# JTtNinjaCode/CPU-Ray-Tracing-Implementation

Hardware: AMD Instinct MI355X
Metric: Msamples/sec (pixels*spp) Cornell Box 800x800@1024spp; 1/2/4/8-GPU scaling (higher is better)
Workload: dtype fp64; 1 GPU; cornell_box 800x800 1024spp depth 50, light sampling on; key=cornell_box 800x800 1024spp depth 50 f64 pool=0 chunk=0 K=0 world=1, spp=1024, max_depth=50, tiles=16x16 round-robin over ranks, parallelism=tiles1, kernel_timing=on, rounds_per_frame=1, grid_lanes=458752

## Files before the change

### cpu-ray-tracing-implementation_amd/csrc/rt_device.h

```cpp
#pragma once

#include <hip/hip_runtime.h>
#include <stdint.h>

#include <type_traits>

#include "rt_scene.h"
#include "rt_sin.h"
#include "rt_types.h"

namespace rtd {

#ifndef RT_BIG_SPHERE_R
#define RT_BIG_SPHERE_R 16
#endif
#define RT_EXT_FN __device__ __attribute__((noinline))

#ifndef RT_PRECISE_F32
__device__ __forceinline__ float fdiv(float a, float b) { return a * __builtin_amdgcn_rcpf(b); }
__device__ __forceinline__ float fsqrt(float x) { return __builtin_amdgcn_sqrtf(x); }
__device__ __forceinline__ float flog(float x) { return __builtin_amdgcn_logf(x) * 0.693147180559945309f; }
__device__ __forceinline__ float frsq(float x) { return __builtin_amdgcn_rsqf(x); }
__device__ __forceinline__ void sincos2pi(float u, float& s, float& c) {
  s = __builtin_amdgcn_sinf(u);
  c = __builtin_amdgcn_cosf(u);
}
#else
__device__ __forceinline__ float fdiv(float a, float b) { return a / b; }
__device__ __forceinline__ float fsqrt(float x) { return sqrtf(x); }
__device__ __forceinline__ float flog(float x) { return logf(x); }
__device__ __forceinline__ float frsq(float x) { return 1.0f / sqrtf(x); }
__device__ __forceinline__ void sincos2pi(float u, float& s, float& c) {
  float phi = 2 * 3.14159265358979f * u;
  s = sinf(phi);
  c = cosf(phi);
}
#endif
__device__ __forceinline__ double frcp(double b) {
  const double r0 = __builtin_amdgcn_rcp(b);
// ... 1316 lines not shown
__device__ __forceinline__ void flat_quads(const FlatQuadT<R>* q, uint32_t n, int32_t base, V<R> o, V<R> d,
                                           V<R> inv, R tmin, R& tmax, int32_t& best, uint64_t xkey) {
#pragma unroll 1
  for (uint32_t k = 0; k + 1 < n; k += 2) {
    const FlatQuad2<R> r = ld_scalar(reinterpret_cast<const FlatQuad2<R>*>(q + k));
    flat_quad_test<A>(r.a, base + (int32_t)k, o, d, inv, tmin, tmax, best, xkey);
    flat_quad_test<A>(r.b, base + (int32_t)k + 1, o, d, inv, tmin, tmax, best, xkey);
  }
  if (n & 1u) flat_quad_test<A>(ld_scalar(q + (n - 1)), base + (int32_t)(n - 1), o, d, inv, tmin, tmax, best, xkey);
}
template <class R>
struct Slab {
  R t0[3], t1[3], tn, tf, th;
};
template <class R>
__device__ __forceinline__ Slab<R> flat_slab(const FlatBoxT<R>& b, V<R> o, V<R> inv, R tmin, int32_t excl_i,
                                             uint32_t xf) {
  Slab<R> s;
  const bool left = sizeof(R) == 4 && excl_i == b.inst;
  const R ninf = -Num<R>::inf();
  auto dist = [&](R p, R oa, R ia) { return (p - oa) * ia; };
  s.t0[0] = (left & (xf == 0)) ? ninf : dist(b.lo[0], o.x, inv.x);
  s.t1[0] = (left & (xf == 1)) ? ninf : dist(b.hi[0], o.x, inv.x);
  s.t0[1] = (left & (xf == 2)) ? ninf : dist(b.lo[1], o.y, inv.y);
  s.t1[1] = (left & (xf == 3)) ? ninf : dist(b.hi[1], o.y, inv.y);
  s.t0[2] = (left & (xf == 4)) ? ninf : dist(b.lo[2], o.z, inv.z);
  s.t1[2] = (left & (xf == 5)) ? ninf : dist(b.hi[2], o.z, inv.z);
  s.tn = fmax(fmax(fmin(s.t0[0], s.t1[0]), fmin(s.t0[1], s.t1[1])), fmin(s.t0[2], s.t1[2]));
  s.tf = fmin(fmin(fmax(s.t0[0], s.t1[0]), fmax(s.t0[1], s.t1[1])), fmax(s.t0[2], s.t1[2]));
  s.th = s.tn >= tmin ? s.tn : s.tf;
  return s;
}
template <class R>
__device__ __forceinline__ void trace_flat(const DevScene<R>& sc, V<R> o, V<R> d, uint32_t excl_e, int32_t excl_i,
                                           R& t_best, uint32_t& e_best, int32_t& i_best, uint32_t& nm,
                                           const FlatQuadT<R>* fq, const FlatBoxT<R>* fb) {
  const R tmin = R(0.001);
  R tmax = Num<R>::inf();
  const V<R> inv = flat_inv(d);
  const uint64_t xkey = ((uint64_t)(uint32_t)excl_i << 32) | excl_e;
  const uint32_t xf = excl_e & 7u;
  int32_t best = -1;
  const uint32_t n0 = sc.n_flatq[0], n1 = sc.n_flatq[1], n2 = sc.n_flatq[2], nq = n0 + n1 + n2;
  flat_quads<0>(sc.flatq, n0, 0, o, d, inv, tmin, tmax, best, xkey);
  flat_quads<1>(sc.flatq + n0, n1, (int32_t)n0, o, d, inv, tmin, tmax, best, xkey);
  flat_quads<2>(sc.flatq + n0 + n1, n2, (int32_t)(n0 + n1), o, d, inv, tmin, tmax, best, xkey);
#pragma unroll 1
  for (uint32_t k = 0; k < sc.n_flatb; k++) {
    const FlatBoxT<R> b = ld_scalar(sc.flatb + k);
    const Slab<R> s = flat_slab(b, o, inv, tmin, excl_i, xf);
    const bool h = (s.tf >= fmax(s.tn, tmin)) & (s.th <= tmax);
    tmax = h ? s.th : tmax;
    best = h ? (int32_t)(nq + k) : best;
  }
  t_best = tmax;
  e_best = kNoHit;
  i_best = -1;
  nm = 0;
  if (best < 0) return;
  if ((uint32_t)best < nq) {
    const FlatQuadT<R>& r = fq[best];
    e_best = r.e;
    i_best = r.inst;
    nm = r.nm;
    return;
  }
  const FlatBoxT<R>& b = fb[(uint32_t)best - nq];
  const Slab<R> s = flat_slab(b, o, inv, tmin, excl_i, xf);
  const bool enter = s.tn >= tmin;
  int k = 2;
  if (enter) {
    if (s.tn == fmin(s.t0[0], s.t1[0])) k = 0;
    else if (s.tn == fmin(s.t0[1], s.t1[1])) k = 1;
  } else {
    if (s.tf == fmax(s.t0[0], s.t1[0])) k = 0;
    else if (s.tf == fmax(s.t0[1], s.t1[1])) k = 1;
  }
  const R dk = k == 0 ? d.x : (k == 1 ? d.y : d.z);
  const int side = enter ? (dk < R(0) ? 1 : 0) : (dk < R(0) ? 0 : 1);
  e_best = b.face[2 * k + side];
  i_best = b.inst;
  nm = b.mat | (uint32_t)k << 28 | ((b.neg >> (2 * k + side)) & 1u) << 31;
}

__device__ __forceinline__ double perlin_noise(const double* tb, double px, double py, double pz) {
#pragma clang fp contract(off)
  int iu = (int)floor(px), iv = (int)floor(py), iw = (int)floor(pz);
  const double u = px - iu, v = py - iv, w = pz - iw;
  iu &= 255;
  iv &= 255;
  iw &= 255;
  const double* perm = tb + 3 * kPerlinPoints;
  const double uu = u * u * (3 - 2 * u), vv = v * v * (3 - 2 * v), ww = w * w * (3 - 2 * w);
  double accum = 0.0;
  for (int i = 0; i < 2; i++)
    for (int j = 0; j < 2; j++)
      for (int k = 0; k < 2; k++) {
        const int g = (int)perm[(iu + i) % 256] ^ (int)perm[(iv + j) % 256] ^ (int)perm[(iw + k) % 256];
        const double* r = tb + 3 * g;
        const double d = r[0] * (u - i) + r[1] * (v - j) + r[2] * (w - k);
// ... 266 lines not shown
```

### cpu-ray-tracing-implementation_amd/csrc/rt_kernels.hip

```cpp
#include <hip/hip_runtime.h>

#include <algorithm>
#include <cmath>
#include <map>
#include <mutex>
#include <tuple>

#include "../../include/rt_hip.h"
#include "rt_device.h"
#include "rt_launch.h"

using namespace rtd;

namespace {

#ifndef RT_LINEAR_WAVES
#define RT_LINEAR_WAVES 6
#endif
#ifndef RT_STACK_WAVES
#define RT_STACK_WAVES 4
#endif
#ifndef RT_LINEAR_WAVES_F64
#define RT_LINEAR_WAVES_F64 3
#endif
// ... 719 lines not shown
  static constexpr int kWaves = sizeof(R) != 4 ? (VOL ? RT_LINEAR_VOL_WAVES_F64 : RT_LINEAR_WAVES_F64)
                                 : (!SPH && !TRI && !VOL) ? RT_LINEAR_WAVES
                                 : (!SPH && !TRI && VOL)  ? (LLI ? RT_LINEAR_VOL_WAVES_LLI : RT_LINEAR_VOL_WAVES)
                                                          : 1;
  static constexpr bool kNoRad = VOL;
  static constexpr bool kColdLds = VOL;
  static constexpr bool kThrLds = VOL && LLI && sizeof(R) == 4;
  template <class PS>
  __device__ __forceinline__ static void run(const DevScene<R>& sc, const Node<R>*, const PS& s, Keys k,
                                             uint32_t*, R& t, uint32_t& e, int32_t& i, uint32_t&) {
    trace_linear<R, SPH, TRI, VOL>(sc, s.o, s.d, s.tm, s.xe, s.xi, k, (uint32_t)s.bounce, t, e, i);
  }
};
#ifndef RT_FLAT_WAVES
#define RT_FLAT_WAVES 8
#endif
#ifndef RT_FLAT_WAVES_F64
#define RT_FLAT_WAVES_F64 5
#endif
#ifndef RT_FLAT_WAVES_F64_LL
#define RT_FLAT_WAVES_F64_LL 7
#endif
template <class R, bool TLDS = false, bool LL = false>
struct FlatTrav : TravDefaults {
  static constexpr bool kFlat = true;
  static constexpr bool kTablesLds = TLDS;
  static constexpr bool kLL = LL;
  static constexpr int kWaves = sizeof(R) == 4 ? RT_FLAT_WAVES : (LL ? RT_FLAT_WAVES_F64_LL : RT_FLAT_WAVES_F64);
  static constexpr bool kNoRad = true;
  static constexpr bool kColdLds = sizeof(R) == 8;
  template <class PS>
  __device__ __forceinline__ static void run(const DevScene<R>& sc, const Node<R>*, const PS& s, Keys, uint32_t*,
                                             R& t, uint32_t& e, int32_t& i, uint32_t& nm) {
    trace_flat<R>(sc, s.o, s.d, s.xe, s.xi, t, e, i, nm, sc.flatq, sc.flatb);
  }
  static constexpr uint32_t kLdsQuads = LL ? 16 : 64, kLdsBoxes = LL ? 8 : 16, kLdsMats = LL ? 16 : 32;
  struct Tables {
    FlatQuadT<R> q[kLdsQuads];
    FlatBoxT<R> b[kLdsBoxes];
    Material<R> m[LL ? 1 : kLdsMats];
    R4<R> lm[LL ? kLdsMats : 1];
  };
  __host__ __device__ __forceinline__ static bool tables_fit(const DevScene<R>& sc) {
    return sc.n_flatq[0] + sc.n_flatq[1] + sc.n_flatq[2] <= kLdsQuads && sc.n_flatb <= kLdsBoxes &&
           sc.n_mats <= kLdsMats;
  }
  __device__ __forceinline__ static void fill(const DevScene<R>& sc, Tables& tb) {
    const uint32_t nq = sc.n_flatq[0] + sc.n_flatq[1] + sc.n_flatq[2];
    for (uint32_t j = threadIdx.x; j < nq; j += kBlock) tb.q[j] = sc.flatq[j];
    for (uint32_t j = threadIdx.x; j < sc.n_flatb; j += kBlock) tb.b[j] = sc.flatb[j];
    for (uint32_t j = threadIdx.x; j < sc.n_mats; j += kBlock) {
      if constexpr (LL) {
        const Material<R>& m = sc.mats[j];
        tb.lm[j] = R4<R>{m.tx.c0[0], m.tx.c0[1], m.tx.c0[2], m.kind == M_DIFFUSE_LIGHT ? R(1) : R(0)};
      } else {
        tb.m[j] = sc.mats[j];
      }
    }
  }
  template <class PS>
  __device__ __forceinline__ static void run_lds(const DevScene<R>& sc, const Tables& tb, const PS& s, R& t,
                                                 uint32_t& e, int32_t& i, uint32_t& nm) {
    trace_flat<R>(sc, s.o, s.d, s.xe, s.xi, t, e, i, nm, tb.q, tb.b);
  }
};
constexpr uint32_t kLdsNodeMax = 256;
template <class R, int STACK, bool LDSN = false>
struct StackTrav : TravDefaults {
  static constexpr int kStack = STACK;
  static constexpr int kLdsNodes = LDSN ? (int)kLdsNodeMax : 0;
  static constexpr int kWaves = sizeof(R) == 4 ? RT_STACK_WAVES : (LDSN ? 1 : RT_STACK_WAVES_F64);
  template <class PS>
  __device__ __forceinline__ static void run(const DevScene<R>& sc, const Node<R>* nodes, const PS& s, Keys k,
                                             uint32_t* stk, R& t, uint32_t& e, int32_t& i, uint32_t&) {
    trace<R, STACK, kBlock>(sc, LDSN ? nodes : sc.nodes, s.o, s.d, s.tm, s.xe, s.xi, k, (uint32_t)s.bounce, s.xy(),
                            stk, t, e, i);
  }
};

#ifndef RT_WIDE_WAVES
#define RT_WIDE_WAVES 7
#endif
#ifndef RT_SHADE_BATCH
#define RT_SHADE_BATCH 48
#endif
#ifndef RT_SHADE_BATCH_GLOBAL
#define RT_SHADE_BATCH_GLOBAL 48
#endif
#ifndef RT_WIDE_WAVES_F64
#define RT_WIDE_WAVES_F64 4
#endif
#ifndef RT_WIDE_WAVES_GLOBAL_F64
#define RT_WIDE_WAVES_GLOBAL_F64 4
#endif
#ifndef RT_WIDE_WAVES_GLOBAL_F64_LL
#define RT_WIDE_WAVES_GLOBAL_F64_LL 5
// ... 1074 lines not shown
```

### cpu-ray-tracing-implementation_amd/csrc/rt_render.hip

```cpp
#include <hip/hip_runtime.h>

#include <algorithm>
#include <chrono>
#include <cstdio>
#include <cstdlib>
#include <cstring>
#include <mutex>
#include <new>
#include <stdexcept>
#include <string>
#include <vector>

#include "../../include/rt_hip.h"
#include "rt_launch.h"
#include "rt_plan.h"
#include "scene_compile.h"

using namespace rtd;

struct DevBuf {
  void* ptr = nullptr;
  size_t bytes = 0;
};

// ... 120 lines not shown
    float a = 0;
    RT_HIP(c, hipEventElapsedTime(&a, c->events[k], c->events[k + 1]));
    ms += a;
  }
  c->ev_used = 0;
  c->last.step_ms += ms;
  uint32_t fault = 0;
  if (c->fault.ptr) RT_HIP(c, hipMemcpy(&fault, c->fault.ptr, 4, hipMemcpyDeviceToHost));
  if (fault) return set_err(c, RT_ERR_HIP, "a path did not finish (internal error)");
  return RT_OK;
}

template <class R>
DevScene<R> dev_scene(const SceneHeader& h, void* base) {
  auto at = [&](uint64_t off) { return (const unsigned char*)base + off; };
  DevScene<R> s{};
  s.quads = (const Quad<R>*)at(h.off_quads);
  s.spheres = (const Sphere<R>*)at(h.off_spheres);
  s.tris = (const Tri<R>*)at(h.off_tris);
  s.insts = (const Instance<R>*)at(h.off_instances);
  s.vols = (const Volume<R>*)at(h.off_volumes);
  s.nodes = (const Node<R>*)at(h.off_nodes);
  s.refs = (const uint32_t*)at(h.off_refs);
  s.mats = (const Material<R>*)at(h.off_mats);
  s.texs = (const Texture<R>*)at(h.off_texs);
  s.light = (const Light<R>*)at(h.off_light);
  s.lin = (const LinRec<R>*)at(h.off_linear);
  s.n_linear = h.n_linear;
  s.has_flat = (int32_t)h.has_flat;
  s.flatq = (const FlatQuadT<R>*)at(h.off_flat_quad);
  s.flatb = (const FlatBoxT<R>*)at(h.off_flat_box);
  for (int a = 0; a < 3; a++) s.n_flatq[a] = h.n_flat_quad[a];
  s.n_flatb = h.n_flat_box;
  s.n_mats = h.n_mats;
  s.root = h.root;
  s.background = h.background;
  s.has_volumes = h.has_volumes;
  s.n_nodes = h.n_nodes;
  s.texdata = (const double*)at(h.off_texdata);
  s.images = (const uint8_t*)at(h.off_images);
  s.has_procedural = h.n_texdata > 0 || h.has_cell_noise;
  s.has_wide = (int32_t)h.has_wide;
  s.wnodes = (const WNode*)at(h.off_wnodes);
  s.wprims = (const typename WWord<R>::T*)at(h.off_wprims);
  s.n_wnodes = h.n_wnodes;
  s.n_wprim_words = h.n_wprim_words;
  s.wroot = h.wroot;
  s.wide_stack = h.wide_stack;
  s.wide_kinds = h.wide_kinds;
  s.wide_big = h.wide_big;
  s.wide_top = h.wide_top;
  s.wnodesh = h.has_wnodesh ? (const WNodeH*)at(h.off_wnodesh) : nullptr;
  s.quads64 = h.has_quads64 ? (const Quad<double>*)at(h.off_quads64) : nullptr;
  return s;
}

template <class R>
rt_status wide_spill_area(rt_context* c, const SceneHeader& hdr, DevScene<R>& sc) {
  const uint32_t wide_need = hdr.wide_stack;
  constexpr uint32_t kWideLdsStack = wide_lds_stack<R>();
  if (hdr.has_wide && wide_need > kWideLdsStack) {
    int ncu = 0;
    RT_HIP(c, hipDeviceGetAttribute(&ncu, hipDeviceAttributeMultiprocessorCount, c->device));
    const uint32_t lanes = (uint32_t)std::max(ncu, 1) * 2048u;
    rt_status s;
    if ((s = ensure(c, c->wide_spill, 4ull * (wide_need - kWideLdsStack) * lanes)) != RT_OK) return s;
// ... 728 lines not shown
```

### cpu-ray-tracing-implementation_amd/csrc/rt_scene.h

```cpp
#pragma once

#include <stdint.h>

#if !defined(__HIP__) && !defined(__host__)
#define __host__
#define __device__
#endif

namespace rtd {

enum : uint32_t {
  E_QUAD = 0u,
  E_SPHERE = 1u,
  E_TRI = 2u,
  E_INSTANCE = 3u,
  E_VOLUME = 4u,
  E_NODE = 5u,
  E_LIST = 6u,
  E_SPECIAL = 7u,
};
constexpr uint32_t kTypeShift = 29;
constexpr uint32_t kPayloadMask = (1u << kTypeShift) - 1u;
constexpr uint32_t kEnd = (E_SPECIAL << kTypeShift) | 0u;
constexpr uint32_t kRestoreBase = (E_SPECIAL << kTypeShift) | 1u;
// ... 8 lines not shown
constexpr int kMaxBvhDepth = 26;
constexpr int kLinearMax = 96;
constexpr uint32_t kInstEnd = kRestoreBase;

template <class R>
struct alignas(16) LinRec {
  uint32_t op;
  uint32_t aux;
  R f[14];
};
static_assert(3 * kMaxChain <= 14, "an instance chain must fit one LinRec");

template <class R>
struct alignas(16) FlatQuadT {
  R plane, lo_u, lo_w, inv_u;
  R inv_w;
  uint32_t e;
  int32_t inst;
  uint32_t nm;
};
using FlatQuad = FlatQuadT<float>;
constexpr uint32_t kNmMat = (1u << 28) - 1u;
template <class R>
struct alignas(16) FlatBoxT {
  R lo[3];
  R hi[3];
  int32_t inst;
  uint32_t mat;
  uint32_t face[6];
  uint32_t neg;
  uint32_t pad;
};
using FlatBox = FlatBoxT<float>;
static_assert(sizeof(FlatQuadT<float>) == 32 && sizeof(FlatQuadT<double>) == 64, "flat quad records");
static_assert(sizeof(FlatBoxT<float>) == 64 && sizeof(FlatBoxT<double>) == 96, "flat box records");

template <class R>
struct alignas(16) Quad {
  R n[3];
  R D;
  R q[3];
  int32_t mat;
  R a[3];
  R area;
  R b[3];
  R pad;
};

template <class R>
struct alignas(16) Sphere {
  R c1[3];
  R r;
  R dc[3];
  int32_t mat;
  R cn[3];
  int32_t moving;
};

template <class R>
struct alignas(16) Tri {
  R p0[3];
  int32_t mat;
  R e1[3];
  R pad1;
  R e2[3];
  R pad2;
  R n[3];
// ... 105 lines not shown
  int32_t has_volumes;
  int32_t num_instances;
  uint64_t off_quads, off_spheres, off_tris, off_instances, off_volumes, off_nodes, off_refs, off_mats, off_texs,
      off_light, off_linear;
  uint64_t off_texdata;
  uint64_t n_texdata;
  int32_t has_cell_noise;
  int32_t pad2_;
  uint64_t off_images;
  uint64_t n_images;
  uint64_t bytes;
  uint32_t n_linear;
  uint32_t n_flat_box;
  uint32_t n_flat_quad[3];
  uint32_t has_flat;
  uint64_t off_flat_quad, off_flat_box;
  uint32_t n_quads, n_spheres, n_tris, n_volumes, n_nodes, n_refs, n_mats, n_texs;
  uint64_t off_wnodes, off_wprims;
  uint32_t n_wnodes, n_wprim_words;
  uint32_t wroot;
  uint32_t wide_stack;
  uint32_t wide_kinds;
  uint32_t has_wide;
  uint32_t wide_big;
  uint32_t has_wnodesh;
  uint64_t off_wnodesh;
  uint32_t has_quads64;
  uint64_t off_quads64;
  uint32_t mat_kinds;
  uint32_t tex_kinds;
  int32_t light_kind;
  int32_t light_aligned;
  uint32_t wide_top;
};

}
```

### cpu-ray-tracing-implementation_amd/csrc/rt_types.h

```cpp
#pragma once

#include <hip/hip_runtime.h>
#include <stdint.h>

#include "rt_scene.h"

namespace rtd {

template <class R>
struct V {
  R x, y, z;
};

__host__ __device__ __forceinline__ uint32_t mix32(uint32_t x) {
  x ^= x >> 16;
  x *= 0x21f0aaadu;
  x ^= x >> 15;
  x *= 0xd35a2d97u;
  x ^= x >> 15;
  return x;
}
__host__ __device__ __forceinline__ uint32_t key_pixel(uint64_t seed, uint32_t pixel) {
  return mix32(pixel ^ mix32((uint32_t)seed ^ 0x9E3779B9u));
}
// ... 27 lines not shown
  V<double> pos00;
  V<double> dir;
  V<double> fdir;
  V<double> disk_u, disk_v;
  double focal;
};

template <class R>
struct DevScene {
  const Quad<R>* quads;
  const Sphere<R>* spheres;
  const Tri<R>* tris;
  const Instance<R>* insts;
  const Volume<R>* vols;
  const Node<R>* nodes;
  const uint32_t* refs;
  const Material<R>* mats;
  const Texture<R>* texs;
  const Light<R>* light;
  const LinRec<R>* lin;
  uint32_t n_linear;
  const FlatQuadT<R>* flatq;
  const FlatBoxT<R>* flatb;
  uint32_t n_flatq[3], n_flatb;
  uint32_t n_mats;
  int32_t has_flat;
  uint32_t root;
  int32_t background;
  int32_t has_volumes;
  uint32_t n_nodes;
  const double* texdata;
  const uint8_t* images;
  int32_t has_procedural;
  const WNode* wnodes;
  const typename WWord<R>::T* wprims;
  uint32_t n_wnodes, n_wprim_words, wroot, wide_stack, wide_kinds;
  int32_t has_wide;
  uint32_t wide_big;
  uint32_t wide_top;
  const WNodeH* wnodesh;
  const Quad<double>* quads64;
  const CamDev* cam64;
  uint32_t* wide_spill;
  uint32_t spill_lanes;
};
#ifndef RT_WIDE_TOP_N
#define RT_WIDE_TOP_N 55
#endif
#ifndef RT_WIDE_TOP_N_F64
#define RT_WIDE_TOP_N_F64 85
#endif
#ifndef RT_WIDE_LDS_STACK
#define RT_WIDE_LDS_STACK 12
#endif
#ifndef RT_WIDE_LDS_STACK_F64
#define RT_WIDE_LDS_STACK_F64 18
#endif
template <class R>
constexpr uint32_t wide_lds_stack() {
  return sizeof(R) == 4 ? RT_WIDE_LDS_STACK : RT_WIDE_LDS_STACK_F64;
}

constexpr int kSinCosTab = 1024;

}
```

### cpu-ray-tracing-implementation_amd/csrc/scene_compile.cpp

```cpp
#include "scene_compile.h"

#include <algorithm>
#include <string>
#include <unordered_map>
#include <cmath>
#include <cstdio>
#include <cstdlib>
#include <cstring>
#include <functional>
#include <limits>
#include <new>
#include <stdexcept>

namespace rtd {
namespace {
constexpr int kPermAxes[6][3] = {{2, 0, 1}, {1, 0, 2}, {2, 1, 0}, {0, 1, 2}, {1, 2, 0}, {0, 2, 1}};

constexpr double kInf = std::numeric_limits<double>::infinity();
constexpr int kSmallList = 8;
constexpr int kLeafMax = 4;

struct Box {
  double lo[3] = {kInf, kInf, kInf};
  double hi[3] = {-kInf, -kInf, -kInf};
// ... 120 lines not shown
  Light<double> light_{};
  int depth_guard_ = 0;

  bool fail(const std::string& m) {
    if (ok_) err_ = m;
    ok_ = false;
    return false;
  }
  const rt_object* obj(int i) {
    if (i < 0 || i >= d_->num_objects) {
      fail("object index " + std::to_string(i) + " out of range");
      return nullptr;
    }
    return &d_->objects[i];
  }
  bool check_mat(int m) {
    if (m < 0 || m >= d_->num_materials) return fail("primitive without a valid material");
    return true;
  }
  static bool is_wrapper(int kind) { return kind >= RT_OBJ_TRANSLATE && kind <= RT_OBJ_ROTATE_Z; }
  static Op op_of(const rt_object& o) {
    if (o.kind == RT_OBJ_TRANSLATE) return {0, o.a[0], o.a[1], o.a[2]};
    return {o.kind - RT_OBJ_ROTATE_X + 1, o.s0, o.s1, 0.0};
  }

  Item prim_item(const rt_object& o);
  void gather(int idx, const std::vector<Op>& chain, std::vector<Item>& out, bool ordered_ctx);
  Item container(std::vector<Item>& items, bool ordered);
  Item list_of(const std::vector<Item>& items);
  Item bvh(std::vector<Item>& items, size_t b, size_t e, int depth);
  int make_instance(const std::vector<Op>& chain, uint32_t blas);
  LinRec<double> lin_record(uint32_t op) const;
  bool flat_program(const std::vector<uint32_t>& lin, std::vector<FlatQuadT<double>>& quads, uint32_t nq[3],
                    std::vector<FlatBoxT<double>>& boxes);
  bool wide_bvh(const std::vector<Item>& prims, CompiledScene* out);
  bool box_of_quads(const std::vector<Item>& prims, double lo[3], double hi[3]) const;
  std::vector<int> aligned_;
  std::vector<double> qu_, qv_;
  std::vector<int32_t> quad_obj_, sphere_obj_, tri_obj_, vol_obj_;
  void light_from(int idx);
};

Item Compiler::prim_item(const rt_object& o) {
  Item it{};
  const int32_t oi = (int32_t)(&o - d_->objects);
  it.need = 0;
  it.depth = 0;
  it.volume = false;
  if (!check_mat(o.material)) return it;
  if (o.kind == RT_OBJ_QUAD) {
    Quad<double> q{};
    double n[3], nn;
    v_cross(o.b, o.c, n);
    v_unit(n, q.n);
    q.area = std::sqrt(n[0] * n[0] + n[1] * n[1] + n[2] * n[2]);
    for (int k = 0; k < 3; k++) q.q[k] = o.a[k];
    q.D = v_dot(q.n, q.q);
    nn = v_dot(n, n);
    double w[3] = {n[0] / nn, n[1] / nn, n[2] / nn};
    v_cross(o.c, w, q.a);
    v_cross(w, o.b, q.b);
    q.mat = mat_id(o.material);
    quads_.push_back(q);
    quad_obj_.push_back(oi);
    it.entry = mk(E_QUAD, (uint32_t)quads_.size() - 1);
    auto single_axis = [](const double* v) {
      int k = -1;
// ... 630 lines not shown
      r.f[3] = 1.0 / qu_[i];
      r.f[4] = 1.0 / qv_[i];
      r.f[5] = qu_[i];
      r.f[6] = qv_[i];
    } else {
      for (int k = 0; k < 3; k++) {
        r.f[k] = q.n[k];
        r.f[4 + k] = q.q[k];
        r.f[7 + k] = q.a[k];
        r.f[10 + k] = q.b[k];
      }
      r.f[3] = q.D;
    }
  } else if (ty == E_SPHERE) {
    const Sphere<double>& sp = spheres_[i];
    for (int k = 0; k < 3; k++) {
      r.f[k] = sp.c1[k];
      r.f[4 + k] = sp.dc[k];
    }
    r.f[3] = sp.r;
    r.aux = (uint32_t)sp.moving;
  } else if (ty == E_TRI) {
    const Tri<double>& t = tris_[i];
    for (int k = 0; k < 3; k++) {
      r.f[k] = t.p0[k];
      r.f[3 + k] = t.e1[k];
      r.f[6 + k] = t.e2[k];
    }
  }
  return r;
}

bool Compiler::flat_program(const std::vector<uint32_t>& lin, std::vector<FlatQuadT<double>>& quads, uint32_t nq[3],
                            std::vector<FlatBoxT<double>>& boxes) {
  struct Q {
    uint32_t e;
    int32_t inst;
    int A, U, W;
    double plane, lo_u, lo_w, len_u, len_w;
  };
  auto quad_of = [&](uint32_t op, int32_t inst, Q& q) {
    const uint32_t i = epay(op);
    if (etype(op) != E_QUAD || !aligned_[i]) return false;
    const int* ax = kPermAxes[aligned_[i] - 1];
    q.e = op;
    q.inst = inst;
    q.A = ax[0];
    q.plane = quads_[i].q[ax[0]];
    double lu = quads_[i].q[ax[1]], lv = quads_[i].q[ax[2]], su = qu_[i], sv = qv_[i];
    if (ax[1] < ax[2]) {
      q.U = ax[1], q.W = ax[2], q.lo_u = lu, q.lo_w = lv, q.len_u = su, q.len_w = sv;
    } else {
      q.U = ax[2], q.W = ax[1], q.lo_u = lv, q.lo_w = lu, q.len_u = sv, q.len_w = su;
    }
    return true;
  };
  std::vector<FlatQuadT<double>> grp[3];
  auto add_quad = [&](const Q& q, const double* off) {
    FlatQuadT<double> r{};
    r.plane = q.plane + off[q.A];
    r.lo_u = q.lo_u + off[q.U];
    r.lo_w = q.lo_w + off[q.W];
    r.inv_u = 1.0 / q.len_u;
    r.inv_w = 1.0 / q.len_w;
    r.e = q.e;
    r.inst = q.inst;
    const Quad<double>& qq = quads_[epay(q.e)];
    r.nm = (uint32_t)qq.mat | (uint32_t)q.A << 28 | (qq.n[q.A] < 0 ? 1u << 31 : 0u);
    grp[q.A].push_back(r);
  };
  auto as_box = [&](const std::vector<Q>& qs, const double* off, FlatBoxT<double>& b) {
    if (qs.size() != 6) return false;
    const int32_t mat = quads_[epay(qs[0].e)].mat;
    if (mats_[(size_t)mat].kind != M_LAMBERTIAN) return false;
    double lo[3], hi[3];
    int cnt[3] = {0, 0, 0};
    for (const Q& q : qs) {
      if (quads_[epay(q.e)].mat != mat) return false;
      if (cnt[q.A] == 0) lo[q.A] = hi[q.A] = q.plane;
      lo[q.A] = std::min(lo[q.A], q.plane);
      hi[q.A] = std::max(hi[q.A], q.plane);
      cnt[q.A]++;
    }
    for (int k = 0; k < 3; k++)
      if (cnt[k] != 2 || !(lo[k] < hi[k])) return false;
    int seen[6] = {0, 0, 0, 0, 0, 0};
    for (const Q& q : qs) {
      const double u0 = std::min(q.lo_u, q.lo_u + q.len_u), u1 = std::max(q.lo_u, q.lo_u + q.len_u);
      const double w0 = std::min(q.lo_w, q.lo_w + q.len_w), w1 = std::max(q.lo_w, q.lo_w + q.len_w);
      if (u0 != lo[q.U] || u1 != hi[q.U] || w0 != lo[q.W] || w1 != hi[q.W]) return false;
      const int f = 2 * q.A + (q.plane == hi[q.A] ? 1 : 0);
      if (seen[f]++) return false;
      b.face[f] = q.e;
      if (quads_[epay(q.e)].n[q.A] < 0) b.neg |= 1u << f;
    }
    for (int k = 0; k < 3; k++) {
      b.lo[k] = lo[k] + off[k];
      b.hi[k] = hi[k] + off[k];
    }
    b.inst = qs[0].inst;
    b.mat = (uint32_t)mat;
    return true;
  };
  const double zero[3] = {0, 0, 0};
  const size_t quads_before = quads_.size();
  auto undo = [&]() {
    quads_.resize(quads_before);
    quad_obj_.resize(quads_before);
    aligned_.resize(quads_before);
    qu_.resize(quads_before);
    qv_.resize(quads_before);
    return false;
  };
  for (size_t k = 0; k < lin.size(); k++) {
    const uint32_t op = lin[k];
    if (etype(op) == E_QUAD) {
      Q q;
      if (!quad_of(op, -1, q)) return undo();
      add_quad(q, zero);
      continue;
    }
    if (etype(op) != E_INSTANCE) return undo();
    const int32_t ii = (int32_t)epay(op);
    const Instance<double>& in = insts_[(size_t)ii];
    double off[3] = {0, 0, 0};
    for (int j = 0; j < in.nops; j++) {
      if (in.op[j].kind != 0) return undo();
      off[0] += in.op[j].x;
      off[1] += in.op[j].y;
      off[2] += in.op[j].z;
    }
    std::vector<Q> qs;
    for (k++; k < lin.size() && lin[k] != kInstEnd; k++) {
      Q q;
      if (!quad_of(lin[k], ii, q)) return undo();
      qs.push_back(q);
    }
    if (k == lin.size()) return undo();
    FlatBoxT<double> b{};
    if (as_box(qs, off, b)) {
      while (quads_.size() % 8) {
        quads_.push_back(quads_[0]);
        quad_obj_.push_back(-1);
        aligned_.push_back(aligned_[0]);
        qu_.push_back(qu_[0]);
        qv_.push_back(qv_[0]);
      }
      for (int f = 0; f < 6; f++) {
        const uint32_t i = epay(b.face[f]);
        quads_.push_back(quads_[i]);
        quad_obj_.push_back(quad_obj_[i]);
        aligned_.push_back(aligned_[i]);
        qu_.push_back(qu_[i]);
        qv_.push_back(qv_[i]);
        b.face[f] = mk(E_QUAD, (uint32_t)quads_.size() - 1);
      }
      boxes.push_back(b);
    } else
      for (const Q& q : qs) add_quad(q, off);
  }
  quads.clear();
  for (int a = 0; a < 3; a++) {
    nq[a] = (uint32_t)grp[a].size();
    quads.insert(quads.end(), grp[a].begin(), grp[a].end());
  }
  return true;
}

bool Compiler::box_of_quads(const std::vector<Item>& prims, double lo[3], double hi[3]) const {
  if (prims.size() != 6) return false;
  int cnt[3] = {0, 0, 0};
  for (const Item& it : prims) {
    if (etype(it.entry) != E_QUAD || !aligned_[epay(it.entry)]) return false;
    const int A = kPermAxes[aligned_[epay(it.entry)] - 1][0];
    const double plane = quads_[epay(it.entry)].q[A];
    if (cnt[A] == 0) lo[A] = hi[A] = plane;
    lo[A] = std::min(lo[A], plane);
    hi[A] = std::max(hi[A], plane);
    cnt[A]++;
  }
  for (int k = 0; k < 3; k++)
    if (cnt[k] != 2 || !(lo[k] < hi[k])) return false;
  int faces = 0;
  for (const Item& it : prims) {
    const uint32_t i = epay(it.entry);
    const int* ax = kPermAxes[aligned_[i] - 1];
    const double q[3] = {quads_[i].q[0], quads_[i].q[1], quads_[i].q[2]};
    const double u0 = std::min(q[ax[1]], q[ax[1]] + qu_[i]), u1 = std::max(q[ax[1]], q[ax[1]] + qu_[i]);
    const double v0 = std::min(q[ax[2]], q[ax[2]] + qv_[i]), v1 = std::max(q[ax[2]], q[ax[2]] + qv_[i]);
    if (u0 != lo[ax[1]] || u1 != hi[ax[1]] || v0 != lo[ax[2]] || v1 != hi[ax[2]]) return false;
    faces |= 1 << (2 * ax[0] + (q[ax[0]] == hi[ax[0]] ? 1 : 0));
  }
  return faces == 63;
}

bool Compiler::wide_bvh(const std::vector<Item>& all, CompiledScene* out) {
  std::vector<Item> prims, big;
// ... 421 lines not shown
  }
  if (d_->background >= d_->num_textures) {
    *err = "background texture out of range";
    return false;
  }
  std::vector<Item> top;
  gather(d_->world, {}, top, false);
  if (ok_) light_from(d_->light);
  if (!ok_) {
    *err = err_;
    return false;
  }
  const rt_object* w = &d_->objects[d_->world];
  bool ordered = (w->kind == RT_OBJ_LIST);
  Item root;
  if (top.empty()) {
    root = list_of(top);
  } else if (ordered) {
    root = container(top, false);
  } else {
    root = top.size() == 1 ? top[0] : bvh(top, 0, top.size(), 0);
  }
  if (root.need + 1 > kStackDepth) {
    *err = "scene needs a deeper traversal stack than the device provides";
    return false;
  }
  Item lin_top;
  join_lin(lin_top, top);
  std::vector<LinRec<double>> linear;
  if (lin_top.lin_ok)
    for (uint32_t op : lin_top.lin) linear.push_back(lin_record(op));
  std::vector<FlatQuadT<double>> fq;
  std::vector<FlatBoxT<double>> fb;
  uint32_t nq[3] = {0, 0, 0};
  out->desc_quads = (int)quads_.size();
  const bool has_flat = lin_top.lin_ok && !lin_top.lin.empty() && flat_program(lin_top.lin, fq, nq, fb);
  if (has_flat) {
    for (const FlatQuadT<double>& q : fq) out->flat_quads += q.inst != -2;
    out->flat_boxes = (int)fb.size();
  }
  out->stack_need = std::max(1, root.need);
  out->bvh_depth = root.depth;
  out->num_items = (int)top.size();
  out->hdr64 =
      pack(out->blob64, quads_, spheres_, tris_, insts_, vols_, nodes_, refs_, mats_, texs_, light_, linear, texdata_, images_);
  out->hdr = pack(out->blob32, map32(quads_), map32(spheres_), map32(tris_), map32(insts_), map32(vols_),
                  map32(nodes_), refs_, map32(mats_), map32(texs_), to32(light_), map32(linear), texdata_, images_);
  if (!quads_.empty()) {
    out->hdr.off_quads64 = append(out->blob32, quads_);
    out->hdr.has_quads64 = 1;
    out->blob32.resize((out->blob32.size() + 255) & ~size_t(255));
    out->hdr.bytes = out->blob32.size();
  }
  if (has_flat) {
    std::vector<FlatQuadT<float>> fq32;
    std::vector<FlatBoxT<float>> fb32;
    for (const FlatQuadT<double>& q : fq)
      fq32.push_back({(float)q.plane, (float)q.lo_u, (float)q.lo_w, (float)q.inv_u, (float)q.inv_w, q.e, q.inst, q.nm});
    for (const FlatBoxT<double>& b : fb) {
      FlatBoxT<float> r{};
      for (int k = 0; k < 3; k++) {
        r.lo[k] = (float)b.lo[k];
        r.hi[k] = (float)b.hi[k];
      }
      r.inst = b.inst;
      r.mat = b.mat;
      for (int f = 0; f < 6; f++) r.face[f] = b.face[f];
      r.neg = b.neg;
      fb32.push_back(r);
    }
    auto put = [&](std::vector<unsigned char>& blob, SceneHeader& h, const auto& q, const auto& b) {
      h.off_flat_quad = append(blob, q);
      h.off_flat_box = append(blob, b);
      blob.resize((blob.size() + 255) & ~size_t(255));
      h.bytes = blob.size();
      for (int a = 0; a < 3; a++) h.n_flat_quad[a] = nq[a];
      h.n_flat_box = (uint32_t)b.size();
      h.has_flat = 1;
    };
    put(out->blob32, out->hdr, fq32, fb32);
    put(out->blob64, out->hdr64, fq, fb);
  }
  out->ids.clear();
  uint32_t tab = 0;
  for (const std::vector<int32_t>* v : {&quad_obj_, &sphere_obj_, &tri_obj_, &vol_obj_}) {
    out->ids_off[tab++] = (uint32_t)(out->ids.size() / 2);
    for (int32_t oi : *v) {
      out->ids.push_back(oi);
      out->ids.push_back(oi >= 0 ? d_->objects[oi].material : -1);
    }
  }
  bool prims_only = etype(root.entry) == E_NODE;
  for (const Item& it : top) prims_only = prims_only && etype(it.entry) <= E_TRI;
  if (prims_only && !wide_bvh(top, out)) out->hdr.has_wide = out->hdr64.has_wide = 0;
  for (SceneHeader* h : {&out->hdr, &out->hdr64}) {
    h->has_cell_noise = cell_noise_ ? 1 : 0;
    h->root = root.entry;
    h->background = d_->background;
    h->has_volumes = vols_.empty() ? 0 : 1;
  }
  return true;
}

}

rt_status compile_scene(const rt_scene_desc* desc, CompiledScene* out, std::string* err) {
  if (!desc || !out || !err) return RT_ERR_INVALID_ARGUMENT;
  if (desc->world < 0 || desc->world >= desc->num_objects) {
    *err = "world object index out of range";
    return RT_ERR_INVALID_ARGUMENT;
  }
  try {
    Compiler c(desc);
    if (!c.run(out, err)) return RT_ERR_UNSUPPORTED;
// ... 12 lines not shown
```

### cpu-ray-tracing-implementation_amd/csrc/scene_compile.h

```cpp
#pragma once

#include <stdint.h>

#include <string>
#include <vector>

#include "../../include/rt_hip.h"
#include "rt_scene.h"

namespace rtd {

struct CompiledScene {
  SceneHeader hdr{};
  std::vector<unsigned char> blob32;
  std::vector<unsigned char> blob64;
  SceneHeader hdr64{};
  int stack_need = 0;
  int bvh_depth = 0;
  int num_items = 0;
  int desc_quads = 0;
  int flat_quads = 0, flat_boxes = 0;
  std::vector<int32_t> ids;
  uint32_t ids_off[4] = {0, 0, 0, 0};
};

rt_status compile_scene(const rt_scene_desc* desc, CompiledScene* out, std::string* err);

}
```

Baseline: 26840 Msamples/s.

## Collapse axis-aligned quad groups into slab-tested room records in flat traversal

```diff
diff --git a/cpu-ray-tracing-implementation_amd/csrc/rt_device.h b/cpu-ray-tracing-implementation_amd/csrc/rt_device.h
--- a/cpu-ray-tracing-implementation_amd/csrc/rt_device.h
+++ b/cpu-ray-tracing-implementation_amd/csrc/rt_device.h
@@ -5,6 +5,7 @@
 
 #include <type_traits>
 
+#include "rt_room.h"
 #include "rt_scene.h"
 #include "rt_sin.h"
 #include "rt_types.h"
@@ -1387,9 +1388,26 @@
   return s;
 }
 template <class R>
+__device__ __forceinline__ RoomHit<R> flat_room_test(const FlatRoomHeadT<R>& b, V<R> o, V<R> inv, R tmin,
+                                                     uint32_t excl_e, int32_t excl_i) {
+  auto dist = [&](R p, R oa, R ia) { return (p - oa) * ia; };
+  R t0[3] = {dist(b.lo[0], o.x, inv.x), dist(b.lo[1], o.y, inv.y), dist(b.lo[2], o.z, inv.z)};
+  R t1[3] = {dist(b.hi[0], o.x, inv.x), dist(b.hi[1], o.y, inv.y), dist(b.hi[2], o.z, inv.z)};
+  if constexpr (sizeof(R) == 4) {
+    const bool left = excl_i == b.inst;
+    const R ninf = -Num<R>::inf();
+#pragma unroll
+    for (int k = 0; k < 3; k++) {
+      t0[k] = (left & (excl_e == b.e[2 * k]) & ((b.present >> (2 * k)) & 1u)) ? ninf : t0[k];
+      t1[k] = (left & (excl_e == b.e[2 * k + 1]) & ((b.present >> (2 * k + 1)) & 1u)) ? ninf : t1[k];
+    }
+  }
+  return room_rule<R>(t0, t1, b.present, tmin);
+}
+template <class R>
 __device__ __forceinline__ void trace_flat(const DevScene<R>& sc, V<R> o, V<R> d, uint32_t excl_e, int32_t excl_i,
                                            R& t_best, uint32_t& e_best, int32_t& i_best, uint32_t& nm,
-                                           const FlatQuadT<R>* fq, const FlatBoxT<R>* fb) {
+                                           const FlatQuadT<R>* fq, const FlatRoomT<R>* fr, const FlatBoxT<R>* fb) {
   const R tmin = R(0.001);
   R tmax = Num<R>::inf();
   const V<R> inv = flat_inv(d);
@@ -1400,13 +1418,23 @@
   flat_quads<0>(sc.flatq, n0, 0, o, d, inv, tmin, tmax, best, xkey);
   flat_quads<1>(sc.flatq + n0, n1, (int32_t)n0, o, d, inv, tmin, tmax, best, xkey);
   flat_quads<2>(sc.flatq + n0 + n1, n2, (int32_t)(n0 + n1), o, d, inv, tmin, tmax, best, xkey);
+  const uint32_t nr8 = (sizeof(R) == 8 || kFlatRoomsF32) ? 8u * sc.n_flatr : 0u;
+  const FlatRoomT<R>* rooms = flat_rooms(sc);
+#pragma unroll 1
+  for (uint32_t k = 0; k < nr8; k += 8u) {
+    const FlatRoomHeadT<R> b = ld_scalar(reinterpret_cast<const FlatRoomHeadT<R>*>(rooms + (k >> 3)));
+    const RoomHit<R> r = flat_room_test(b, o, inv, tmin, excl_e, excl_i);
+    const bool h = r.hit & (r.t <= tmax);
+    tmax = h ? r.t : tmax;
+    best = h ? (int32_t)(nq + k) + r.face : best;
+  }
 #pragma unroll 1
   for (uint32_t k = 0; k < sc.n_flatb; k++) {
     const FlatBoxT<R> b = ld_scalar(sc.flatb + k);
     const Slab<R> s = flat_slab(b, o, inv, tmin, excl_i, xf);
     const bool h = (s.tf >= fmax(s.tn, tmin)) & (s.th <= tmax);
     tmax = h ? s.th : tmax;
-    best = h ? (int32_t)(nq + k) : best;
+    best = h ? (int32_t)(nq + nr8 + k) : best;
   }
   t_best = tmax;
   e_best = kNoHit;
@@ -1420,7 +1448,15 @@
     nm = r.nm;
     return;
   }
-  const FlatBoxT<R>& b = fb[(uint32_t)best - nq];
+  if ((uint32_t)best < nq + nr8) {
+    const uint32_t j = (uint32_t)best - nq;
+    const FlatRoomT<R>& r = fr[j >> 3];
+    e_best = r.e[j & 7u];
+    i_best = r.inst;
+    nm = r.nm[j & 7u];
+    return;
+  }
+  const FlatBoxT<R>& b = fb[(uint32_t)best - nq - nr8];
   const Slab<R> s = flat_slab(b, o, inv, tmin, excl_i, xf);
   const bool enter = s.tn >= tmin;
   int k = 2;
diff --git a/cpu-ray-tracing-implementation_amd/csrc/rt_kernels.hip b/cpu-ray-tracing-implementation_amd/csrc/rt_kernels.hip
--- a/cpu-ray-tracing-implementation_amd/csrc/rt_kernels.hip
+++ b/cpu-ray-tracing-implementation_amd/csrc/rt_kernels.hip
@@ -775,22 +775,26 @@
   template <class PS>
   __device__ __forceinline__ static void run(const DevScene<R>& sc, const Node<R>*, const PS& s, Keys, uint32_t*,
                                              R& t, uint32_t& e, int32_t& i, uint32_t& nm) {
-    trace_flat<R>(sc, s.o, s.d, s.xe, s.xi, t, e, i, nm, sc.flatq, sc.flatb);
-  }
-  static constexpr uint32_t kLdsQuads = LL ? 16 : 64, kLdsBoxes = LL ? 8 : 16, kLdsMats = LL ? 16 : 32;
+    trace_flat<R>(sc, s.o, s.d, s.xe, s.xi, t, e, i, nm, sc.flatq, flat_rooms(sc), sc.flatb);
+  }
+  static constexpr uint32_t kLdsQuads = LL ? 14 : 64, kLdsBoxes = LL ? 8 : 16, kLdsMats = LL ? 16 : 32;
+  static constexpr uint32_t kLdsRooms = LL ? 1 : 2;
   struct Tables {
     FlatQuadT<R> q[kLdsQuads];
+    FlatRoomT<R> r[kLdsRooms];
     FlatBoxT<R> b[kLdsBoxes];
     Material<R> m[LL ? 1 : kLdsMats];
     R4<R> lm[LL ? kLdsMats : 1];
   };
   __host__ __device__ __forceinline__ static bool tables_fit(const DevScene<R>& sc) {
     return sc.n_flatq[0] + sc.n_flatq[1] + sc.n_flatq[2] <= kLdsQuads && sc.n_flatb <= kLdsBoxes &&
-           sc.n_mats <= kLdsMats;
+           sc.n_flatr <= kLdsRooms && sc.n_mats <= kLdsMats;
   }
   __device__ __forceinline__ static void fill(const DevScene<R>& sc, Tables& tb) {
     const uint32_t nq = sc.n_flatq[0] + sc.n_flatq[1] + sc.n_flatq[2];
     for (uint32_t j = threadIdx.x; j < nq; j += kBlock) tb.q[j] = sc.flatq[j];
+    if constexpr (sizeof(R) == 8 || kFlatRoomsF32)
+      for (uint32_t j = threadIdx.x; j < sc.n_flatr; j += kBlock) tb.r[j] = flat_rooms(sc)[j];
     for (uint32_t j = threadIdx.x; j < sc.n_flatb; j += kBlock) tb.b[j] = sc.flatb[j];
     for (uint32_t j = threadIdx.x; j < sc.n_mats; j += kBlock) {
       if constexpr (LL) {
@@ -804,7 +808,7 @@
   template <class PS>
   __device__ __forceinline__ static void run_lds(const DevScene<R>& sc, const Tables& tb, const PS& s, R& t,
                                                  uint32_t& e, int32_t& i, uint32_t& nm) {
-    trace_flat<R>(sc, s.o, s.d, s.xe, s.xi, t, e, i, nm, tb.q, tb.b);
+    trace_flat<R>(sc, s.o, s.d, s.xe, s.xi, t, e, i, nm, tb.q, tb.r, tb.b);
   }
 };
 constexpr uint32_t kLdsNodeMax = 256;
diff --git a/cpu-ray-tracing-implementation_amd/csrc/rt_render.hip b/cpu-ray-tracing-implementation_amd/csrc/rt_render.hip
--- a/cpu-ray-tracing-implementation_amd/csrc/rt_render.hip
+++ b/cpu-ray-tracing-implementation_amd/csrc/rt_render.hip
@@ -176,6 +176,7 @@
   s.flatb = (const FlatBoxT<R>*)at(h.off_flat_box);
   for (int a = 0; a < 3; a++) s.n_flatq[a] = h.n_flat_quad[a];
   s.n_flatb = h.n_flat_box;
+  s.n_flatr = h.n_flat_room;
   s.n_mats = h.n_mats;
   s.root = h.root;
   s.background = h.background;
diff --git a/cpu-ray-tracing-implementation_amd/csrc/rt_room.h b/cpu-ray-tracing-implementation_amd/csrc/rt_room.h
--- /dev/null
+++ b/cpu-ray-tracing-implementation_amd/csrc/rt_room.h
@@ -0,0 +1,59 @@
+#pragma once
+
+#include <math.h>
+#include <stdint.h>
+
+#if !defined(__HIP__) && !defined(__host__)
+#define __host__
+#define __device__
+#endif
+
+namespace rtd {
+
+constexpr uint32_t kRoomAllFaces = 63u;
+
+__host__ __device__ inline uint32_t room_absent(uint32_t present) {
+  uint32_t f = 0;
+  while (f < 6u && ((present >> f) & 1u)) f++;
+  return f;
+}
+__host__ __device__ inline bool room_mask_ok(uint32_t present) {
+  const uint32_t miss = ~present & kRoomAllFaces;
+  return (present & ~kRoomAllFaces) == 0 && (miss & (miss - 1u)) == 0;
+}
+
+template <class R>
+struct RoomHit {
+  bool hit;
+  R t;
+  int face;
+};
+
+template <class R>
+__host__ __device__ inline RoomHit<R> room_rule(const R t0[3], const R t1[3], uint32_t present, R tmin) {
+  const R n0 = fmin(t0[0], t1[0]), n1 = fmin(t0[1], t1[1]), n2 = fmin(t0[2], t1[2]);
+  const R f0 = fmax(t0[0], t1[0]), f1 = fmax(t0[1], t1[1]), f2 = fmax(t0[2], t1[2]);
+  const R tn = fmax(fmax(n0, n1), n2);
+  const R tf = fmin(fmin(f0, f1), f2);
+  bool in_absent = false, out_absent = false;
+  switch (room_absent(present)) {
+    case 0: in_absent = tn == t0[0], out_absent = tf == t0[0]; break;
+    case 1: in_absent = tn == t1[0], out_absent = tf == t1[0]; break;
+    case 2: in_absent = tn == t0[1], out_absent = tf == t0[1]; break;
+    case 3: in_absent = tn == t1[1], out_absent = tf == t1[1]; break;
+    case 4: in_absent = tn == t0[2], out_absent = tf == t0[2]; break;
+    case 5: in_absent = tn == t1[2], out_absent = tf == t1[2]; break;
+    default: break;
+  }
+  const bool enter = (tn >= tmin) & !in_absent;
+  RoomHit<R> r;
+  r.hit = (tf >= fmax(tn, tmin)) & (enter | !out_absent);
+  r.t = enter ? tn : tf;
+  const bool l0 = t0[0] == r.t, h0 = t1[0] == r.t, l1 = t0[1] == r.t, h1 = t1[1] == r.t, h2 = t1[2] == r.t;
+  const bool a0 = l0 | h0, a1 = l1 | h1;
+  const bool hi = (a0 & h0) | (!a0 & a1 & h1) | (!a0 & !a1 & h2);
+  r.face = (a0 ? 0 : (a1 ? 2 : 4)) + (hi ? 1 : 0);
+  return r;
+}
+
+}
diff --git a/cpu-ray-tracing-implementation_amd/csrc/rt_scene.h b/cpu-ray-tracing-implementation_amd/csrc/rt_scene.h
--- a/cpu-ray-tracing-implementation_amd/csrc/rt_scene.h
+++ b/cpu-ray-tracing-implementation_amd/csrc/rt_scene.h
@@ -64,7 +64,28 @@
   uint32_t pad;
 };
 using FlatBox = FlatBoxT<float>;
+template <class R>
+struct alignas(16) FlatRoomHeadT {
+  R lo[3];
+  R hi[3];
+  int32_t inst;
+  uint32_t present;
+  uint32_t e[6];
+};
+template <class R>
+struct alignas(16) FlatRoomT {
+  R lo[3];
+  R hi[3];
+  int32_t inst;
+  uint32_t present;
+  uint32_t e[6];
+  uint32_t nm[6];
+};
+using FlatRoom = FlatRoomT<float>;
+constexpr bool kFlatRoomsF32 = false;
 static_assert(sizeof(FlatQuadT<float>) == 32 && sizeof(FlatQuadT<double>) == 64, "flat quad records");
+static_assert(sizeof(FlatRoomT<float>) == 80 && sizeof(FlatRoomT<double>) == 112, "flat room records");
+static_assert(sizeof(FlatRoomHeadT<float>) == 64 && sizeof(FlatRoomHeadT<double>) == 80, "flat room heads");
 static_assert(sizeof(FlatBoxT<float>) == 64 && sizeof(FlatBoxT<double>) == 96, "flat box records");
 
 template <class R>
@@ -236,6 +257,8 @@
   int32_t light_kind;
   int32_t light_aligned;
   uint32_t wide_top;
+  uint32_t n_flat_room;
+  uint64_t off_flat_room;
 };
 
 }
diff --git a/cpu-ray-tracing-implementation_amd/csrc/rt_types.h b/cpu-ray-tracing-implementation_amd/csrc/rt_types.h
--- a/cpu-ray-tracing-implementation_amd/csrc/rt_types.h
+++ b/cpu-ray-tracing-implementation_amd/csrc/rt_types.h
@@ -83,6 +83,7 @@
   const double* texdata;
   const uint8_t* images;
   int32_t has_procedural;
+  uint32_t n_flatr;
   const WNode* wnodes;
   const typename WWord<R>::T* wprims;
   uint32_t n_wnodes, n_wprim_words, wroot, wide_stack, wide_kinds;
@@ -95,6 +96,10 @@
   uint32_t* wide_spill;
   uint32_t spill_lanes;
 };
+template <class R>
+__host__ __device__ __forceinline__ const FlatRoomT<R>* flat_rooms(const DevScene<R>& sc) {
+  return reinterpret_cast<const FlatRoomT<R>*>(sc.flatb + sc.n_flatb);
+}
 #ifndef RT_WIDE_TOP_N
 #define RT_WIDE_TOP_N 55
 #endif
diff --git a/cpu-ray-tracing-implementation_amd/csrc/scene_compile.cpp b/cpu-ray-tracing-implementation_amd/csrc/scene_compile.cpp
--- a/cpu-ray-tracing-implementation_amd/csrc/scene_compile.cpp
+++ b/cpu-ray-tracing-implementation_amd/csrc/scene_compile.cpp
@@ -176,7 +176,8 @@
   int make_instance(const std::vector<Op>& chain, uint32_t blas);
   LinRec<double> lin_record(uint32_t op) const;
   bool flat_program(const std::vector<uint32_t>& lin, std::vector<FlatQuadT<double>>& quads, uint32_t nq[3],
-                    std::vector<FlatBoxT<double>>& boxes);
+                    std::vector<FlatBoxT<double>>& boxes, std::vector<FlatRoomT<double>>& rooms,
+                    std::vector<FlatQuadT<double>>& quads_all, uint32_t nq_all[3]);
   bool wide_bvh(const std::vector<Item>& prims, CompiledScene* out);
   bool box_of_quads(const std::vector<Item>& prims, double lo[3], double hi[3]) const;
   std::vector<int> aligned_;
@@ -873,7 +874,8 @@
 }
 
 bool Compiler::flat_program(const std::vector<uint32_t>& lin, std::vector<FlatQuadT<double>>& quads, uint32_t nq[3],
-                            std::vector<FlatBoxT<double>>& boxes) {
+                            std::vector<FlatBoxT<double>>& boxes, std::vector<FlatRoomT<double>>& rooms,
+                            std::vector<FlatQuadT<double>>& quads_all, uint32_t nq_all[3]) {
   struct Q {
     uint32_t e;
     int32_t inst;
@@ -896,8 +898,12 @@
     }
     return true;
   };
-  std::vector<FlatQuadT<double>> grp[3];
-  auto add_quad = [&](const Q& q, const double* off) {
+  std::vector<FlatQuadT<double>> grp[3], grp_all[3];
+  auto nm_of = [&](const Q& q) {
+    const Quad<double>& qq = quads_[epay(q.e)];
+    return (uint32_t)qq.mat | (uint32_t)q.A << 28 | (qq.n[q.A] < 0 ? 1u << 31 : 0u);
+  };
+  auto add_quad = [&](const Q& q, const double* off, bool in_room) {
     FlatQuadT<double> r{};
     r.plane = q.plane + off[q.A];
     r.lo_u = q.lo_u + off[q.U];
@@ -906,9 +912,73 @@
     r.inv_w = 1.0 / q.len_w;
     r.e = q.e;
     r.inst = q.inst;
-    const Quad<double>& qq = quads_[epay(q.e)];
-    r.nm = (uint32_t)qq.mat | (uint32_t)q.A << 28 | (qq.n[q.A] < 0 ? 1u << 31 : 0u);
-    grp[q.A].push_back(r);
+    r.nm = nm_of(q);
+    grp_all[q.A].push_back(r);
+    if (!in_room) grp[q.A].push_back(r);
+  };
+  struct Pending {
+    Q q;
+    double off[3];
+    int pool;
+    bool in_room;
+  };
+  std::vector<Pending> pend;
+  int pools = 1;
+  auto span = [](double a, double len, double& s0, double& s1) { s0 = std::min(a, a + len), s1 = std::max(a, a + len); };
+  auto extent = [&](const Q& q, int k, double& s0, double& s1) {
+    if (k == q.U) span(q.lo_u, q.len_u, s0, s1);
+    else span(q.lo_w, q.len_w, s0, s1);
+  };
+  auto find_rooms = [&](int pool) {
+    std::vector<size_t> ix;
+    for (size_t k = 0; k < pend.size(); k++)
+      if (pend[k].pool == pool) ix.push_back(k);
+    for (size_t i : ix) {
+      if (pend[i].in_room) continue;
+      const Q& a = pend[i].q;
+      for (size_t j : ix) {
+        const Q& b = pend[j].q;
+        if (pend[i].in_room) break;
+        if (j == i || pend[j].in_room || b.A == a.A) continue;
+        double lo[3], hi[3];
+        extent(a, a.U, lo[a.U], hi[a.U]);
+        extent(a, a.W, lo[a.W], hi[a.W]);
+        extent(b, a.A, lo[a.A], hi[a.A]);
+        if (!(lo[0] < hi[0] && lo[1] < hi[1] && lo[2] < hi[2])) continue;
+        size_t face[6];
+        uint32_t present = 0;
+        bool twice = false;
+        for (size_t k : ix) {
+          const Q& q = pend[k].q;
+          if (pend[k].in_room || (q.plane != lo[q.A] && q.plane != hi[q.A])) continue;
+          double u0, u1, w0, w1;
+          extent(q, q.U, u0, u1);
+          extent(q, q.W, w0, w1);
+          if (u0 != lo[q.U] || u1 != hi[q.U] || w0 != lo[q.W] || w1 != hi[q.W]) continue;
+          const int f = 2 * q.A + (q.plane == hi[q.A] ? 1 : 0);
+          twice = twice || ((present >> f) & 1u);
+          present |= 1u << f;
+          face[f] = k;
+        }
+        int n = 0;
+        for (int f = 0; f < 6; f++) n += (present >> f) & 1u;
+        if (twice || n < 5 || !((present >> (2 * a.A + (a.plane == hi[a.A] ? 1 : 0))) & 1u)) continue;
+        FlatRoomT<double> r{};
+        for (int k = 0; k < 3; k++) {
+          r.lo[k] = lo[k] + pend[i].off[k];
+          r.hi[k] = hi[k] + pend[i].off[k];
+        }
+        r.inst = a.inst;
+        r.present = present;
+        for (int f = 0; f < 6; f++) {
+          if (!((present >> f) & 1u)) continue;
+          r.e[f] = pend[face[f]].q.e;
+          r.nm[f] = nm_of(pend[face[f]].q);
+          pend[face[f]].in_room = true;
+        }
+        rooms.push_back(r);
+      }
+    }
   };
   auto as_box = [&](const std::vector<Q>& qs, const double* off, FlatBoxT<double>& b) {
     if (qs.size() != 6) return false;
@@ -943,7 +1013,6 @@
     b.mat = (uint32_t)mat;
     return true;
   };
-  const double zero[3] = {0, 0, 0};
   const size_t quads_before = quads_.size();
   auto undo = [&]() {
     quads_.resize(quads_before);
@@ -958,7 +1027,7 @@
     if (etype(op) == E_QUAD) {
       Q q;
       if (!quad_of(op, -1, q)) return undo();
-      add_quad(q, zero);
+      pend.push_back({q, {0, 0, 0}, 0, false});
       continue;
     }
     if (etype(op) != E_INSTANCE) return undo();
@@ -997,13 +1066,20 @@
         b.face[f] = mk(E_QUAD, (uint32_t)quads_.size() - 1);
       }
       boxes.push_back(b);
-    } else
-      for (const Q& q : qs) add_quad(q, off);
-  }
+    } else {
+      for (const Q& q : qs) pend.push_back({q, {off[0], off[1], off[2]}, pools, false});
+      pools++;
+    }
+  }
+  for (int p = 0; p < pools; p++) find_rooms(p);
+  for (const Pending& p : pend) add_quad(p.q, p.off, p.in_room);
   quads.clear();
+  quads_all.clear();
   for (int a = 0; a < 3; a++) {
     nq[a] = (uint32_t)grp[a].size();
     quads.insert(quads.end(), grp[a].begin(), grp[a].end());
+    nq_all[a] = (uint32_t)grp_all[a].size();
+    quads_all.insert(quads_all.end(), grp_all[a].begin(), grp_all[a].end());
   }
   return true;
 }
@@ -1491,12 +1567,17 @@
     for (uint32_t op : lin_top.lin) linear.push_back(lin_record(op));
   std::vector<FlatQuadT<double>> fq;
   std::vector<FlatBoxT<double>> fb;
-  uint32_t nq[3] = {0, 0, 0};
+  std::vector<FlatRoomT<double>> fr;
+  std::vector<FlatQuadT<double>> fq_all;
+  uint32_t nq[3] = {0, 0, 0}, nq_all[3] = {0, 0, 0};
   out->desc_quads = (int)quads_.size();
-  const bool has_flat = lin_top.lin_ok && !lin_top.lin.empty() && flat_program(lin_top.lin, fq, nq, fb);
+  const bool has_flat =
+      lin_top.lin_ok && !lin_top.lin.empty() && flat_program(lin_top.lin, fq, nq, fb, fr, fq_all, nq_all);
   if (has_flat) {
-    for (const FlatQuadT<double>& q : fq) out->flat_quads += q.inst != -2;
+    out->flat_quads = (int)fq_all.size();
     out->flat_boxes = (int)fb.size();
+    out->flat_rooms = (int)fr.size();
+    for (const FlatRoomT<double>& r : fr) out->room_masks.push_back(r.present);
   }
   out->stack_need = std::max(1, root.need);
   out->bvh_depth = root.depth;
@@ -1514,8 +1595,21 @@
   if (has_flat) {
     std::vector<FlatQuadT<float>> fq32;
     std::vector<FlatBoxT<float>> fb32;
-    for (const FlatQuadT<double>& q : fq)
+    std::vector<FlatRoomT<float>> fr32;
+    for (const FlatQuadT<double>& q : kFlatRoomsF32 ? fq : fq_all)
       fq32.push_back({(float)q.plane, (float)q.lo_u, (float)q.lo_w, (float)q.inv_u, (float)q.inv_w, q.e, q.inst, q.nm});
+    for (const FlatRoomT<double>& b : fr) {
+      if (!kFlatRoomsF32) break;
+      FlatRoomT<float> r{};
+      for (int k = 0; k < 3; k++) {
+        r.lo[k] = (float)b.lo[k];
+        r.hi[k] = (float)b.hi[k];
+      }
+      r.inst = b.inst;
+      r.present = b.present;
+      for (int f = 0; f < 6; f++) r.e[f] = b.e[f], r.nm[f] = b.nm[f];
+      fr32.push_back(r);
+    }
     for (const FlatBoxT<double>& b : fb) {
       FlatBoxT<float> r{};
       for (int k = 0; k < 3; k++) {
@@ -1528,17 +1622,23 @@
       r.neg = b.neg;
       fb32.push_back(r);
     }
-    auto put = [&](std::vector<unsigned char>& blob, SceneHeader& h, const auto& q, const auto& b) {
+    auto put = [&](std::vector<unsigned char>& blob, SceneHeader& h, const auto& q, const uint32_t* n, const auto& b,
+                   const auto& r) {
       h.off_flat_quad = append(blob, q);
-      h.off_flat_box = append(blob, b);
+      std::vector<unsigned char> br(b.size() * sizeof(b[0]) + r.size() * sizeof(r[0]));
+      if (!b.empty()) memcpy(br.data(), b.data(), b.size() * sizeof(b[0]));
+      if (!r.empty()) memcpy(br.data() + b.size() * sizeof(b[0]), r.data(), r.size() * sizeof(r[0]));
+      h.off_flat_box = append(blob, br);
+      h.off_flat_room = h.off_flat_box + b.size() * sizeof(b[0]);
       blob.resize((blob.size() + 255) & ~size_t(255));
       h.bytes = blob.size();
-      for (int a = 0; a < 3; a++) h.n_flat_quad[a] = nq[a];
+      for (int a = 0; a < 3; a++) h.n_flat_quad[a] = n[a];
       h.n_flat_box = (uint32_t)b.size();
+      h.n_flat_room = (uint32_t)r.size();
       h.has_flat = 1;
     };
-    put(out->blob32, out->hdr, fq32, fb32);
-    put(out->blob64, out->hdr64, fq, fb);
+    put(out->blob32, out->hdr, fq32, kFlatRoomsF32 ? nq : nq_all, fb32, fr32);
+    put(out->blob64, out->hdr64, fq, nq, fb, fr);
   }
   out->ids.clear();
   uint32_t tab = 0;
diff --git a/cpu-ray-tracing-implementation_amd/csrc/scene_compile.h b/cpu-ray-tracing-implementation_amd/csrc/scene_compile.h
--- a/cpu-ray-tracing-implementation_amd/csrc/scene_compile.h
+++ b/cpu-ray-tracing-implementation_amd/csrc/scene_compile.h
@@ -20,6 +20,8 @@
   int num_items = 0;
   int desc_quads = 0;
   int flat_quads = 0, flat_boxes = 0;
+  int flat_rooms = 0;
+  std::vector<uint32_t> room_masks;
   std::vector<int32_t> ids;
   uint32_t ids_off[4] = {0, 0, 0, 0};
 };
```

Result: faster. 27570 Msamples/s (median of 6 runs) (+2.7%).
